# Monash-Connected-Autonomous-Vehicle/unsupervised-pseuso-LiDAR

Measured on AMD Instinct MI355X. Metric: images/sec (fwd+bwd) KITTI 192x640 triplets, full training step, higher is better.
Workload: dtype f32; 1 GPU; BASELINE.json configs[1]: per-GPU batch=12, 192x640 KITTI-shaped triplets, ResNet-18 depth encoder + 6-DoF PoseNet, fp32 (the ResNet trunk's 3x3 stride-1 convolutions and their data gradients: fp32 contractions on split operands -- three bf16 planes per operand, six bf16-MFMA plane products, fp32 accumulation; every other launch: fp32 MFMA), one step = 2x depth fwd + pose fwd + warp/L1/smooth loss; global_batch=12, parallelism=dp1

## Files before the change

### unsupervised-pseuso-lidar_amd/csrc/conv_igemm.hip

```cpp
#include <stdlib.h>
#include <map>
#include <mutex>
#include <type_traits>
#include <utility>

#include "conv_shared.h"
#include "kernel_timer.h"

namespace mcav {

template <class T, int KIND>
__global__ __launch_bounds__(256) void igemm_kernel(IgemmParams p) {
    constexpr int BM = T::BM, BN = T::BN;
    constexpr int CK = T::KD;
    __shared__ __attribute__((aligned(16))) float As[2][BM][T::LD];
    __shared__ __attribute__((aligned(16))) float Bs[2][BN][T::LD];
    __shared__ int s_out[BM];
    __shared__ float s_stat[T::WAVES_M][2][BN];
    constexpr int MAXTAB = 9;
    __shared__ unsigned s_o1[KIND == K_GENERIC ? 1 : MAXTAB][KIND == K_GENERIC ? 1 : BM];
    __shared__ unsigned s_o2[KIND == K_GENERIC ? 1 : MAXTAB][KIND == K_GENERIC ? 1 : BM];
    __shared__ int s_rn[KIND == K_GENERIC ? 1 : BM], s_ry[KIND == K_GENERIC ? 1 : BM], s_rx[KIND == K_GENERIC ? 1 : BM];

    const int tid = threadIdx.x, lane = tid & 63, wave = tid >> 6;
// ... 1251 lines not shown
        maybe_build(t + 1); step(B1{}, B0{}, F1{}, ra0, rb0);
        maybe_build(t + 2); step(B0{}, B1{}, F1{}, ra1, rb1);
        maybe_build(t + 3); step(B1{}, B0{}, F0{}, ra0, rb0);
    } else if (rest == 3) {
        maybe_build(t);     step(B0{}, B1{}, F1{}, ra1, rb1);
        maybe_build(t + 1); step(B1{}, B0{}, F1{}, ra0, rb0);
        maybe_build(t + 2); step(B0{}, B1{}, F0{}, ra1, rb1);
    } else if (rest == 2) {
        maybe_build(t);     step(B0{}, B1{}, F1{}, ra1, rb1);
        maybe_build(t + 1); step(B1{}, B0{}, F0{}, ra0, rb0);
    } else if (rest == 1) {
        maybe_build(t);     step(B0{}, B1{}, F0{}, ra1, rb1);
    }

    constexpr int MF = T::MF;
    const int ccol = lane & (MF - 1);
    float* slab = p.slab + (size_t)split * (p.Ktot + 1) * p.slabN;
    if (do_bias) {
        if (bpix < BPIX) *reinterpret_cast<f32x4*>(&Ys[0][bpix][bcol * 4]) = bsum;
        __syncthreads();
        if (tid < BN) {
            float tsum = 0.f;
            for (int k = 0; k < BPIX; ++k) tsum += Ys[0][k][tid];
            if (n0 + tid < p.slabN) slab[(size_t)p.Ktot * p.slabN + n0 + tid] = tsum;
        }
    }
    const __amdgpu_buffer_rsrc_t rslab = make_rsrc(slab, (unsigned)((size_t)p.Ktot * p.slabN * 4));
    const int rowb = p.slabN * 4;
#pragma unroll
    for (int i = 0; i < T::TM; ++i)
#pragma unroll
        for (int j = 0; j < T::TN; ++j) {
            const int n = n0 + wn0 + j * MF + ccol;
            if (n < p.slabN) {
                const unsigned base = (unsigned)(m0 + wm0 + i * MF + (MF == 32 ? 4 * (lane >> 5) : 4 * (lane >> 4))) * (unsigned)rowb + (unsigned)n * 4u;
#pragma unroll
                for (int r = 0; r < T::ACC; ++r) {
                    const int dr = MF == 32 ? (r & 3) + 8 * (r >> 2) : r;
                    buf_store1(rslab, base + (unsigned)(dr * rowb), acc[i][j][r]);
                }
            }
        }
}

__device__ __forceinline__ void wgrad_presum_body(const float* slab, int splits, size_t elems, int per_group, float* dst, unsigned bx, unsigned by) {
    const size_t e4 = (size_t)bx * 256 + threadIdx.x;
    if (e4 * 4 >= elems) return;
    const int k0 = by * per_group, k1 = min(splits, k0 + per_group);
    const f32x4* src = reinterpret_cast<const f32x4*>(slab) + e4;
    const size_t stride4 = elems / 4;
    f32x4 s0 = {0.f, 0.f, 0.f, 0.f}, s1 = s0, s2 = s0, s3 = s0;
    int k = k0;
    for (; k + 3 < k1; k += 4) {
        s0 += src[(size_t)k * stride4];
        s1 += src[(size_t)(k + 1) * stride4];
        s2 += src[(size_t)(k + 2) * stride4];
        s3 += src[(size_t)(k + 3) * stride4];
    }
    for (; k < k1; ++k) s0 += src[(size_t)k * stride4];
    reinterpret_cast<f32x4*>(dst)[(size_t)by * stride4 + e4] = (s0 + s1) + (s2 + s3);
}

__global__ __launch_bounds__(256) void wgrad_presum_kernel(const float* slab, int splits, size_t elems, int per_group, float* dst) {
    wgrad_presum_body(slab, splits, elems, per_group, dst, blockIdx.x, blockIdx.y);
}

__device__ __forceinline__ void wgrad_reduce_body(float* lds, const float* slab, int splits, int Ktot, int slabN, int Kp, int taps, int Cout, int Cin,
                                                  int CI_T, float* dw, float* dbias, int accumulate, int upm, int Cin_total, int ci_off, int bx, int by) {
    const int co0 = bx * 32, ci0 = by * CI_T;
    const int tx = threadIdx.x & 31, ty = threadIdx.x >> 5;
    const int run = CI_T * taps, stride = run + 1;
    const size_t split_stride = (size_t)(Ktot + 1) * slabN;
    const bool col_ok = co0 + tx < slabN;
    if (upm) {
        for (int idx = ty; idx < run; idx += 8) {
            const int tap = idx / CI_T, r = idx - tap * CI_T, ci = ci0 + r;
            float sum = 0.f;
            if (ci < Cin && col_ok) {
                const int ky = tap / 3, kx = tap - ky * 3;
                for (int cls = 0; cls < 4; ++cls) {
                    const int py = cls >> 1, px = cls & 1;
                    const int ta = py == 0 ? (ky == 0 ? 0 : 1) : (ky == 2 ? 1 : 0), tb = px == 0 ? (kx == 0 ? 0 : 1) : (kx == 2 ? 1 : 0);
                    const float* src = slab + (size_t)((cls * 4 + ta * 2 + tb) * Kp + ci) * slabN + co0 + tx;
                    for (int k = 0; k < splits; ++k) sum += src[(size_t)k * split_stride];
                }
            }
            lds[tx * stride + r * taps + tap] = sum;
        }
    } else {
        for (int idx0 = ty; idx0 < run; idx0 += 32) {
            const float* src[4];
            float sum[4];
            int at[4];
#pragma unroll
            for (int u = 0; u < 4; ++u) {
                const int idx = idx0 + 8 * u, tap = idx / CI_T, r = idx - tap * CI_T;
                const bool ok = idx < run && ci0 + r < Cin && col_ok;
                src[u] = ok ? slab + (size_t)(tap * Kp + ci0 + r) * slabN + co0 + tx : nullptr;
                at[u] = idx < run ? tx * stride + r * taps + tap : -1;
                sum[u] = 0.f;
            }
            int k = 0;
            for (; k + 3 < splits; k += 4) {
                float v[4][4];
#pragma unroll
                for (int u = 0; u < 4; ++u)
#pragma unroll
                    for (int j = 0; j < 4; ++j) v[u][j] = src[u] ? src[u][(size_t)(k + j) * split_stride] : 0.f;
#pragma unroll
                for (int u = 0; u < 4; ++u)
#pragma unroll
                    for (int j = 0; j < 4; ++j) sum[u] += v[u][j];
            }
            for (; k < splits; ++k) {
#pragma unroll
                for (int u = 0; u < 4; ++u) sum[u] += src[u] ? src[u][(size_t)k * split_stride] : 0.f;
            }
#pragma unroll
            for (int u = 0; u < 4; ++u)
                if (at[u] >= 0) lds[at[u]] = sum[u];
        }
    }
    if (dbias && by == 0 && ty == 0 && co0 + tx < Cout) {
        const float* src = slab + (size_t)Ktot * slabN + co0 + tx;
        float sum = 0.f;
        for (int k = 0; k < splits; ++k) sum += src[(size_t)k * split_stride];
        dbias[co0 + tx] = accumulate ? dbias[co0 + tx] + sum : sum;
    }
    __syncthreads();
    const int valid_run = (Cin - ci0 < CI_T ? Cin - ci0 : CI_T) * taps;
    for (int e = threadIdx.x; e < 32 * run; e += 256) {
        const int col = e / run, q = e - col * run;
        if (co0 + col < Cout && q < valid_run) {
            const size_t o = ((size_t)(co0 + col) * Cin_total + ci_off + ci0) * taps + q;
            const float v = lds[col * stride + q];
            dw[o] = accumulate ? dw[o] + v : v;
        }
    }
}

__global__ __launch_bounds__(256) void wgrad_reduce_kernel(const float* slab, int splits, int Ktot, int slabN, int Kp, int taps, int Cout, int Cin,
                                                           int CI_T, float* dw, float* dbias, int accumulate, int upm, int Cin_total, int ci_off) {
    extern __shared__ float lds[];
    wgrad_reduce_body(lds, slab, splits, Ktot, slabN, Kp, taps, Cout, Cin, CI_T, dw, dbias, accumulate, upm, Cin_total, ci_off, blockIdx.x, blockIdx.y);
}

__device__ __forceinline__ int find_item(const mcav_wgrad_reduce_item* items, int n, int blk, bool presum) {
    int lo = 0;
    for (int i = 1; i < n; ++i)
        if ((presum ? items[i].pre_first : items[i].red_first) <= blk) lo = i;
    return lo;
}

__global__ __launch_bounds__(256) void wgrad_presum_multi_kernel(const mcav_wgrad_reduce_item* items, int n) {
    __shared__ int s_i;
    if (threadIdx.x == 0) {
        int best = -1;
        for (int i = 0; i < n; ++i)
            if (items[i].groups > 0 && items[i].pre_first <= (int)blockIdx.x) best = i;
        s_i = best;
    }
    __syncthreads();
    if (s_i < 0) return;
    const mcav_wgrad_reduce_item it = items[s_i];
    const int local = (int)blockIdx.x - it.pre_first;
    if (local >= it.pre_bx * it.groups) return;
    wgrad_presum_body(it.slab, it.splits, (size_t)it.elems, it.per_group, it.pre, (unsigned)(local % it.pre_bx), (unsigned)(local / it.pre_bx));
}

__global__ __launch_bounds__(256) void wgrad_reduce_multi_kernel(const mcav_wgrad_reduce_item* items, int n) {
    extern __shared__ float lds[];
    __shared__ int s_i;
    if (threadIdx.x == 0) s_i = find_item(items, n, (int)blockIdx.x, false);
    __syncthreads();
    const mcav_wgrad_reduce_item it = items[s_i];
    const int local = (int)blockIdx.x - it.red_first;
    if (local >= it.red_gx * it.red_gy) return;
    const float* src = it.groups > 0 ? it.pre : it.slab;
    wgrad_reduce_body(lds, src, it.groups > 0 ? it.groups : it.splits, it.Ktot, it.slabN, it.Kp, it.taps, it.Cout, it.Cin, it.ci_t, it.dw, it.dbias,
                      it.accumulate, it.upm, it.cin_total, it.ci_off, local % it.red_gx, local / it.red_gx);
}

__global__ void pack_weights_kernel(const float* w, int Cout, int Cin, int taps, int transposed, float* packed, int Np, int Kp, int Kstride) {
    const size_t total = (size_t)Np * Kstride;
    for (size_t e = (size_t)blockIdx.x * blockDim.x + threadIdx.x; e < total; e += (size_t)gridDim.x * blockDim.x) {
        const int n = (int)(e / Kstride), kf = (int)(e - (size_t)n * Kstride);
        const int tap = kf / Kp, k = kf - tap * Kp;
        float v = 0.f;
        if (tap < taps) {
            const int co = transposed ? k : n, ci = transposed ? n : k;
            if (co < Cout && ci < Cin) v = w[((size_t)co * Cin + ci) * taps + tap];
        }
        packed[e] = v;
    }
}

struct PackItem {
    const float* src;
    float* dst;
    int Cout, Cin, taps, transposed, Np, Kp, Kstride, first_block;
};

constexpr int PK_LDS = 5120;
constexpr int PK_CO = 64;

__host__ __device__ inline int pack_ci_tile(int taps) { const int t = 79 / taps; return t < 1 ? 1 : (t > 8 ? 8 : t); }

constexpr int PK_MERGE = 2048;

__device__ __forceinline__ float upmerge_elem(const float* w, int Cout, int Cin, int C1, int Np, size_t e) {
    const int c = (int)(e % C1);
    const int mt = (int)((e / C1) % 4), n = (int)((e / ((size_t)C1 * 4)) % Np), cls = (int)(e / ((size_t)C1 * 4 * Np));
    const int py = cls >> 1, px = cls & 1, a = mt >> 1, b = mt & 1;
    float sum = 0.f;
    if (n < Cout) {
        const float* wc = w + ((size_t)n * Cin + c) * 9;
        for (int ky = 0; ky < 3; ++ky)
            for (int kx = 0; kx < 3; ++kx) {
                const bool iny = py == 0 ? (a == 0 ? ky == 0 : ky >= 1) : (a == 0 ? ky <= 1 : ky == 2);
                const bool inx = px == 0 ? (b == 0 ? kx == 0 : kx >= 1) : (b == 0 ? kx <= 1 : kx == 2);
                if (iny && inx) sum += wc[ky * 3 + kx];
            }
    }
    return sum;
}

__device__ __forceinline__ float upmerge_adj_elem(const float* w, int Cout, int Cin, int C1, int Kp, size_t e) {
    const int k = (int)(e % Kp), tap = (int)((e / Kp) % 16), n = (int)(e / ((size_t)Kp * 16));
    const int u = tap >> 2, v = tap & 3;
    float sum = 0.f;
    if (n < C1 && k < Cout) {
        const float* wc = w + ((size_t)k * Cin + n) * 9;
        for (int ky = 0; ky < 3; ++ky)
            for (int kx = 0; kx < 3; ++kx) {
                const bool iny = u == 0 ? ky == 2 : (u == 1 ? ky >= 1 : (u == 2 ? ky <= 1 : ky == 0));
                const bool inx = v == 0 ? kx == 2 : (v == 1 ? kx >= 1 : (v == 2 ? kx <= 1 : kx == 0));
                if (iny && inx) sum += wc[ky * 3 + kx];
            }
    }
    return sum;
}

__host__ __device__ inline size_t pack_merge_total(int transposed, int c1, int Np, int Kp) {
    return (transposed & 16) ? (size_t)Np * 16 * Kp : (size_t)4 * Np * 4 * c1;
}

__host__ __device__ inline int pack_blocks(int transposed, int taps, int Np, int Kp) {
    if (transposed & 24) return (int)((pack_merge_total(transposed, taps, Np, Kp) + PK_MERGE - 1) / PK_MERGE);
    if (!(transposed & 1)) return Np;
    const int ct = pack_ci_tile(taps);
    return ((Np + ct - 1) / ct) * ((Kp + PK_CO - 1) / PK_CO);
}

__global__ __launch_bounds__(256) void pack_weights_multi_kernel(const PackItem* items, int nitems) {
    __shared__ float buf[PK_LDS];
    int lo = 0, hi = nitems - 1;
    while (lo < hi) {
        const int mid = (lo + hi + 1) >> 1;
        if (items[mid].first_block <= (int)blockIdx.x) lo = mid; else hi = mid - 1;
    }
    PackItem it = items[lo];
    if (it.transposed & 24) {
        const size_t total = pack_merge_total(it.transposed, it.taps, it.Np, it.Kp);
        const size_t e0 = (size_t)(blockIdx.x - it.first_block) * PK_MERGE;
        for (int k = 0; k < PK_MERGE / 256; ++k) {
            const size_t e = e0 + (size_t)k * 256 + threadIdx.x;
            if (e < total)
                it.dst[e] = (it.transposed & 16) ? upmerge_adj_elem(it.src, it.Cout, it.Cin, it.taps, it.Kp, e)
                                                 : upmerge_elem(it.src, it.Cout, it.Cin, it.taps, it.Np, e);
        }
        return;
    }
    const bool to_bf16 = (it.transposed & 6) != 0;
    const bool planes = (it.transposed & 4) != 0;
    it.transposed &= 1;
    __bf16* const dst16 = reinterpret_cast<__bf16*>(it.dst);
    const size_t plane = (size_t)it.Np * it.Kstride;
    auto put16 = [&](size_t o, float v) {
        const __bf16 h = (__bf16)v;
        dst16[o] = h;
        if (planes) {
            const float r1 = v - (float)h;
            const __bf16 m = (__bf16)r1;
            dst16[plane + o] = m;
            dst16[2 * plane + o] = (__bf16)(r1 - (float)m);
        }
    };
    const int bl = blockIdx.x - it.first_block, tid = threadIdx.x;
    if (!it.transposed) {
        const int n = bl, run = it.Cin * it.taps;
        float* drow = it.dst + (size_t)n * it.Kstride;
        const bool staged = run <= PK_LDS;
        if (n < it.Cout && staged) {
            const float* srow = it.src + (size_t)n * run;
            for (int q = tid; q < run; q += 256) buf[q] = srow[q];
        }
        __syncthreads();
        for (int kf = tid; kf < it.Kstride; kf += 256) {
            const int tap = kf / it.Kp, k = kf - tap * it.Kp;
            float v = 0.f;
            if (n < it.Cout && tap < it.taps && k < it.Cin) v = staged ? buf[k * it.taps + tap] : it.src[((size_t)n * it.Cin + k) * it.taps + tap];
            if (to_bf16) put16((size_t)n * it.Kstride + kf, v);
            else drow[kf] = v;
        }
        return;
    }
    const int ct = pack_ci_tile(it.taps), run = ct * it.taps, ld = run + 1;
    const int cob = (it.Kp + PK_CO - 1) / PK_CO;
    const int ci0 = (bl / cob) * ct, co0 = (bl % cob) * PK_CO;
    for (int e = tid; e < PK_CO * run; e += 256) {
        const int co = e / run, q = e - co * run;
        float v = 0.f;
        if (co0 + co < it.Cout && ci0 + q / it.taps < it.Cin) v = it.src[((size_t)(co0 + co) * it.Cin + ci0) * it.taps + q];
        buf[co * ld + q] = v;
    }
    __syncthreads();
    for (int e = tid; e < PK_CO * run; e += 256) {
        const int q = e / PK_CO, co = e - q * PK_CO;
        const int r = q / it.taps, tap = q - r * it.taps;
        if (ci0 + r < it.Np && co0 + co < it.Kp) {
            const size_t o = (size_t)(ci0 + r) * it.Kstride + tap * it.Kp + co0 + co;
            if (to_bf16) put16(o, buf[co * ld + q]);
            else it.dst[o] = buf[co * ld + q];
        }
    }
}

__global__ __launch_bounds__(256) void splitk_finish_kernel(const float* __restrict__ slab, int splits, size_t n, int Cd, float* __restrict__ y,
                                                            const float* __restrict__ bias, int n_begin, int act, const float* __restrict__ dact_aux,
                                                            int dact, const float* __restrict__ addend) {
    for (size_t i = (size_t)blockIdx.x * 256 + threadIdx.x; i < n; i += (size_t)gridDim.x * 256) {
        float v = 0.f;
        for (int k = 0; k < splits; ++k) v += slab[(size_t)k * n + i];
        if (bias) v += bias[n_begin + (int)(i % (size_t)Cd)];
        v = act_fwd(v, act);
        if (dact_aux && !(dact & MCAV_DACT_AFTER_ADDEND)) v *= act_bwd(dact_aux[i], dact & 0xff);
        if (addend) v += addend[i];
        if (dact_aux && (dact & MCAV_DACT_AFTER_ADDEND)) v *= act_bwd(dact_aux[i], dact & 0xff);
        y[i] = v;
    }
}

inline float* ksplit_slab(hipStream_t s, size_t bytes) {
    static std::mutex mu;
    static std::map<hipStream_t, std::pair<void*, size_t>> slabs;
    std::lock_guard<std::mutex> lock(mu);
    auto& e = slabs[s];
    if (e.second < bytes) {
        hipStreamCaptureStatus st = hipStreamCaptureStatusNone;
        if (hipStreamIsCapturing(s, &st) != hipSuccess) return nullptr;
        if (st != hipStreamCaptureStatusNone) {
            for (auto& kv : slabs)
                if (kv.second.second >= bytes) return reinterpret_cast<float*>(kv.second.first);
            return nullptr;
        }
        void* ptr = nullptr;
        if (hipMalloc(&ptr, bytes) != hipSuccess) return nullptr;
        e = {ptr, bytes};
    }
    return reinterpret_cast<float*>(e.first);
}

template <class T, int ID>
inline void launch_igemm(const IgemmRoute& r, hipStream_t s) {
    static_assert(T::BM == tile_bm(ID) && T::BN == tile_bn(ID) && T::KD == tile_kd(ID) && T::AROWS == tile_arows(ID), "conv_plan.h's tile table");
    IgemmParams p = r.p;
    if (r.ksplit > 1) {
        float* slab = ksplit_slab(s, (size_t)p.g.B * p.Hd * p.Wd * p.Cd * 4 * r.ksplit);
        if (slab) { p.ksplit = r.ksplit; p.kslab = slab; }
    }
    const int grid = p.mtiles * p.ntiles * p.ksplit;
    const size_t tab_bytes = sizeof(unsigned) * (size_t)p.taps * T::BM * (p.g.C2 > 0 ? 2 : 1);
    const size_t refl_bytes = sizeof(unsigned) * (size_t)p.taps * T::BM * 4;
    switch (r.variant) {
        case MCAV_RV_TABLE | MCAV_RV_UPM: timed_launch(igemm_tab_kernel<T, 2>, grid, dim3(256), sizeof(unsigned) * 13 * T::BM, s, p); break;
        case MCAV_RV_TABLE: timed_launch(igemm_tab_kernel<T, 0>, grid, dim3(256), tab_bytes, s, p); break;
        case MCAV_RV_TABLE | MCAV_RV_REFLECT | MCAV_RV_ADJ: timed_launch(igemm_tab_kernel<T, 1>, grid, dim3(256), refl_bytes, s, p); break;
        case MCAV_RV_FAST: timed_launch(igemm_kernel<T, K_FAST>, grid, dim3(256), 0, s, p); break;
// ... 65 lines not shown
MCAV_EXPORT int mcav_igemm(const mcav_igemm_desc* d, void* stream) {
    IgemmRoute r;
    const int rc = plan_igemm(d, plan_env(), r);
    if (rc != MCAV_OK) return rc;
    hipStream_t s = as_stream(stream);
    switch (r.family) {
        case MCAV_IGEMM_HALO: mcav_halo_launch(r, s); break;
        case MCAV_IGEMM_STEM: mcav_stem_launch(r, s); break;
        case MCAV_IGEMM_FP32:
            switch (r.tile) {
                case 1: launch_igemm<Tile128x64, 1>(r, s); break;
                case 2: launch_igemm<Tile64x64, 2>(r, s); break;
                case 3: launch_igemm<Tile256x32, 3>(r, s); break;
                case 4: launch_igemm<Tile256x16, 4>(r, s); break;
                case 5: launch_igemm<Tile128x128, 5>(r, s); break;
                case 6: launch_igemm<Tile64x16, 6>(r, s); break;
                case 7: launch_igemm<Tile128x32, 7>(r, s); break;
                case 8: launch_igemm<Tile128x64k32, 8>(r, s); break;
                case 9: launch_igemm<Tile128x128k32, 9>(r, s); break;
                case 10: launch_igemm<Tile64x64k32, 10>(r, s); break;
                case 11: launch_igemm<Tile64x64k64, 11>(r, s); break;
                case 12: launch_igemm<Tile32x64k32, 12>(r, s); break;
                default: return MCAV_E_INVALID;
            }
            break;
        default: return mcav_patch_bf16_launch(r, s);
    }
    return launch_status();
}

MCAV_EXPORT int mcav_wgrad_route(const mcav_wgrad_desc* d, mcav_conv_route* out) {
    if (!out) return MCAV_E_INVALID;
    *out = mcav_conv_route{};
    WgradRoute r;
    const int rc = plan_wgrad_route(d, plan_env(), r);
    const WgradParams& p = r.pl.p;
    if (rc == MCAV_OK)
        *out = mcav_conv_route{r.family, r.variant, r.pl.tile, p.mtiles, p.ntiles, r.workgroups, p.splits, r.workspace_bytes()};
    return rc;
}

MCAV_EXPORT size_t mcav_wgrad_workspace_bytes(const mcav_wgrad_desc* d) {
    WgradRoute r;
    return plan_wgrad_route(d, plan_env(), r) == MCAV_OK ? r.workspace_bytes() : 0;
}

MCAV_EXPORT int mcav_wgrad_uses_bf16(const mcav_wgrad_desc* d) {
    WgradRoute r;
    return plan_wgrad_route(d, plan_env(), r) == MCAV_OK && (r.family == MCAV_WGRAD_BF16_PATCH || r.family == MCAV_WGRAD_BF16_TILE);
}

static int wgrad_gemm(const mcav_wgrad_desc* d, void* workspace, size_t workspace_bytes, hipStream_t s, WgradRoute& r) {
    if (plan_wgrad_route(d, plan_env(), r) != MCAV_OK || !workspace) return MCAV_E_INVALID;
    if (workspace_bytes < r.workspace_bytes()) return MCAV_E_WORKSPACE;
    r.pl.p.slab = reinterpret_cast<float*>(workspace);
    switch (r.family) {
        case MCAV_WGRAD_BF16_PATCH:
        case MCAV_WGRAD_BF16_TILE: mcav_bf16_wgrad_launch(r.pl.p, s); break;
        case MCAV_WGRAD_STEM: mcav_stem_wgrad_launch(r, s); break;
        case MCAV_WGRAD_HALO: mcav_halo_wgrad_launch(r, s); break;
        default:
            switch (r.pl.tile) {
                case 1: launch_wgrad<Tile128x64, 1>(r, s); break;
                case 2: launch_wgrad<Tile64x64, 2>(r, s); break;
                case 3: launch_wgrad<Tile256x32, 3>(r, s); break;
                case 4: launch_wgrad<Tile256x16, 4>(r, s); break;
                case 6: launch_wgrad<Tile64x16, 6>(r, s); break;
                case 7: launch_wgrad<Tile128x32, 7>(r, s); break;
                default: return MCAV_E_INVALID;
            }
    }
    return MCAV_OK;
}

static void fill_reduce_item(const mcav_wgrad_desc* d, const WgradPlan& pl, void* workspace, mcav_wgrad_reduce_item& it) {
    it.slab = pl.p.slab;
    it.pre = pl.groups ? reinterpret_cast<float*>(reinterpret_cast<char*>(workspace) + pl.slab_bytes) : nullptr;
    it.dw = d->dw_oihw;
    it.dbias = d->dbias;
    it.elems = (unsigned long long)(pl.p.Ktot + 1) * pl.p.slabN;
    it.splits = pl.p.splits; it.groups = pl.groups; it.per_group = pl.per_group;
    it.Ktot = pl.p.Ktot; it.slabN = pl.p.slabN; it.Kp = pl.p.Kp;
    it.taps = pl.p.upm ? 9 : pl.p.taps;
    it.Cout = d->Cout; it.Cin = d->Cin; it.ci_t = pl.ci_t;
    it.accumulate = d->accumulate; it.upm = pl.p.upm;
    it.cin_total = d->Cin_total > 0 ? d->Cin_total : d->Cin;
    it.ci_off = d->ci_offset;
    it.pre_bx = pl.groups ? (int)((it.elems / 4 + 255) / 256) : 0;
    it.red_gx = (d->Cout + 31) / 32;
    it.red_gy = (d->Cin + pl.ci_t - 1) / pl.ci_t;
    it.pre_first = 0; it.red_first = 0;
}

MCAV_EXPORT int mcav_wgrad(const mcav_wgrad_desc* d, void* workspace, size_t workspace_bytes, void* stream) {
    WgradRoute r;
    hipStream_t s = as_stream(stream);
    const int rc = wgrad_gemm(d, workspace, workspace_bytes, s, r);
    if (rc != MCAV_OK) return rc;
    mcav_wgrad_reduce_item it;
    fill_reduce_item(d, r.pl, workspace, it);
    const size_t lds_bytes = sizeof(float) * 32 * (size_t)(it.ci_t * it.taps + 1);
    const float* rsrc = it.slab;
    int rsplits = it.splits;
    if (it.groups) {
        timed_launch(wgrad_presum_kernel, dim3((unsigned)it.pre_bx, it.groups), dim3(256), 0, s, (const float*)it.slab, it.splits, (size_t)it.elems,
                     it.per_group, it.pre);
// ... 102 lines not shown
```

### unsupervised-pseuso-lidar_amd/mcav/nn.py

```python
import ctypes
import os
import os as _os

import torch

from . import lib as L

c_p, c_i, c_f, c_sz, c_d = L.c_p, L.c_i, L.c_f, L.c_sz, ctypes.c_double

G_DIRECT, G_SMALLC, G_ADJ_REFLECT, G_ADJ_STRIDE2 = 0, 1, 2, 3
PAD_ZERO, PAD_REFLECT = 0, 1
ACT_NONE, ACT_RELU, ACT_ELU, ACT_SIGMOID = 0, 1, 2, 3
DACT_AFTER_ADDEND = 0x100
TILE_ID_MASK = 0xff
TILE_GENERAL = 1 << 9
TILE_HALO_9TAP = 1 << 10
TILE_NO_UPMERGE = 1 << 11
TILE_ALT_UPMERGE = 1 << 12


class IgemmDesc(ctypes.Structure):
    _fields_ = [("x1", c_p), ("x2", c_p), ("B", c_i), ("Hs", c_i), ("Ws", c_i), ("C1", c_i), ("C2", c_i), ("up1", c_i),
                ("w", c_p), ("kh", c_i), ("kw", c_i), ("Np", c_i), ("Kp", c_i),
                ("mode", c_i), ("stride", c_i), ("sign", c_i), ("offset", c_i), ("pad_mode", c_i),
# ... 143 lines not shown
        return False


def _planned(d):
    r = ConvRoute()
    (L.lib().mcav_igemm_route if isinstance(d, IgemmDesc) else L.lib().mcav_wgrad_route)(ctypes.byref(d), ctypes.byref(r))
    return r


def _stem_executed(flops, cout):
    return flops * (8.0 / 7.0) * (1.0 if cout >= 32 else 2.0)


def up16(v):
    return (v + 15) // 16 * 16


def empty(shape, like):
    return torch.empty(shape, dtype=torch.float32, device=like.device)


def P(t):
    return t.data_ptr() if t is not None else None


class _PackItem(ctypes.Structure):
    _fields_ = [("src", c_p), ("dst", c_p), ("Cout", c_i), ("Cin", c_i), ("taps", c_i), ("transposed", c_i), ("Np", c_i), ("Kp", c_i),
                ("Kstride", c_i), ("first_block", c_i)]


MMA_FP32, MMA_BF16, MMA_SPLIT, MMA_SPLIT_ALL = 0, 1, 2, 3
DEFAULT_MMA = MMA_SPLIT
_KINDS = {"f": (False, 0), "b": (True, 0), "f16": (False, 1), "b16": (True, 1), "f16s": (False, 3), "b16s": (True, 3)}


class PackRegistry:

    def __init__(self):
        self.entries = []
        self.table = None
        self.retired = []
        self.nblocks = 0
        self.signature = None

    def add(self, spec, kind):
        import weakref
        self.entries.append((weakref.ref(spec), kind))
        self.signature = None

    def _build(self, device, live):
        items = (_PackItem * len(live))()
        blk = 0
        for it, (spec, kind) in zip(items, live):
            if kind in ("um", "ua"):
                buf = spec._packs[kind]
                it.src, it.dst = spec.weight.data_ptr(), buf.data_ptr()
                it.Cout, it.Cin, it.taps = spec.cout, spec.cin, spec._merge_c1
                if kind == "um":
                    it.transposed, it.Np, it.Kp = 8, spec.np, 0
                else:
                    it.transposed, it.Np, it.Kp = 16, buf.shape[0], buf.shape[1] // 16
                it.Kstride, it.first_block = 0, blk
                blk += L.lib().mcav_pack_weights_blocks(it.taps, it.transposed, it.Np, max(it.Kp, 1))
                continue
            tr, h = _KINDS[kind]
            buf = spec._packs[kind]
            np_, kp_ = (up16(spec.cin), up16(spec.cout)) if tr else (spec.np, spec.kp)
            it.src, it.dst = spec.weight.data_ptr(), buf.data_ptr()
            it.Cout, it.Cin, it.taps, it.transposed = spec.cout, spec.cin, spec.kh * spec.kw, int(tr) | (4 if h == 3 else 2 if h else 0)
            it.Np, it.Kp, it.Kstride, it.first_block = np_, kp_, buf.shape[1], blk
            blk += L.lib().mcav_pack_weights_blocks(it.taps, int(tr), np_, kp_)
        raw = torch.frombuffer(bytearray(bytes(items)), dtype=torch.uint8)
        if self.table is not None:
            self.retired.append(self.table)
        self.table = raw.to(device)
        self.nblocks = blk

    def repack_all(self, device):
        self.entries = [(r, k) for r, k in self.entries if r() is not None]
        live = [(r(), k) for r, k in self.entries]
        live = [(s, k) for s, k in live if s is not None and s.weight.device == device and s._packs.get(k) is not None]
        if not live:
            return
        sig = tuple((s.weight.data_ptr(), s._packs[k].data_ptr()) for s, k in live)
        if self.table is None or sig != self.signature or self.table.device != device:
            self._build(device, live)
            self.signature = sig
        L.check(L.lib().mcav_pack_weights_multi(P(self.table), len(live), self.nblocks, L.stream()), "mcav_pack_weights_multi")
        for s, k in live:
            s._keys[k] = s._key()


PACKS = PackRegistry()


def refresh_packed_weights(device):
    for ref, k in PACKS.entries:
        s = ref()
        if s is None or s.weight.device != device:
            continue
        if s._keys.get(k) != s._key():
            PACKS.repack_all(device)
            return


class ConvSpec:

    def __init__(self, weight, bias, stride, pad, pad_mode, smallc=False):
        self.weight, self.bias = weight, bias
        self.cout, self.cin, self.kh, self.kw = weight.shape
        self.stride, self.pad, self.pad_mode = stride, pad, pad_mode
        self.smallc = smallc
        self.kp = 4 if smallc else up16(self.cin)
        self.np = up16(self.cout)
# ... 8 lines not shown
        tr, h = _KINDS[kind]
        key = self._key()
        buf = self._packs.get(kind)
        if buf is None or self._keys.get(kind) != key or buf.device != self.weight.device:
            taps = self.kh * self.kw
            if buf is None or buf.device != self.weight.device:
                shape = (up16(self.cin), taps * up16(self.cout)) if tr else (self.np, up16(taps * self.kp))
                buf = torch.empty((shape[0] * max(h, 1), shape[1]), dtype=torch.bfloat16 if h else torch.float32, device=self.weight.device)
                f32 = torch.empty(shape, dtype=torch.float32, device=self.weight.device) if h else buf
                np_, kp_ = (up16(self.cin), up16(self.cout)) if tr else (self.np, self.kp)
                L.check(L.lib().mcav_pack_weights(P(self.weight), self.cout, self.cin, self.kh, self.kw, int(tr), P(f32), np_, kp_, L.stream()),
                        "mcav_pack_weights")
                if h == 3:
                    L.check(L.lib().mcav_f32_to_bf16_planes(P(f32), P(buf), f32.numel(), L.stream()), "mcav_f32_to_bf16_planes")
                elif h:
                    L.check(L.lib().mcav_f32_to_bf16(P(f32), P(buf), f32.numel(), L.stream()), "mcav_f32_to_bf16")
                self._packs[kind] = buf
                self._keys[kind] = key
                PACKS.add(self, kind)
            else:
                PACKS.repack_all(self.weight.device)
        return self._packs[kind]

    def packed_fwd(self):
        return self._packed("f")

    def packed_bwd(self):
        return self._packed("b")

    def packed_fwd16(self):
        return self._packed("f16")

    def packed_bwd16(self):
        return self._packed("b16")

    def packed_fwd16s(self):
        return self._packed("f16s")

    def packed_bwd16s(self):
        return self._packed("b16s")

    def is_stem(self):
        return ((self.kh, self.kw, self.stride, self.pad, self.pad_mode) == (7, 7, 2, 3, PAD_ZERO)
                and ((self.smallc and (self.cout, self.cin) == (64, 3)) or (not self.smallc and (self.cout, self.cin) == (16, 9))))

    def takes_stem(self, x2, up1, tile):
        return self.is_stem() and x2 is None and not up1 and not tile & TILE_GENERAL

    def fwd_gather(self):
        return (G_SMALLC if self.smallc else G_DIRECT, self.stride, 1, -self.pad, self.pad_mode)

    def packed_stem(self):
        key = self._key()
        if getattr(self, "_stem", None) is None or self._key_s != key or self._stem.device != self.weight.device:
            if getattr(self, "_stem", None) is None or self._stem.device != self.weight.device:
                self._stem = empty((self.cin * 56, self.cout), self.weight)
            L.check(L.lib().mcav_pack_stem_weights(P(self.weight), self.cout, self.cin, P(self._stem), L.stream()), "mcav_pack_stem_weights")
            self._key_s = key
        return self._stem

    def packed_upmerge(self, c1):
        return self._merged("um", c1, lambda: empty((4, self.np, 4, c1), self.weight),
                            lambda buf: L.lib().mcav_pack_weights_upmerge(P(self.weight), self.cout, self.cin, c1, P(buf), self.np, L.stream()))

    def _merged(self, kind, c1, make, pack):
        key = self._key()
        buf = self._packs.get(kind)
        if buf is None or buf.device != self.weight.device or getattr(self, "_merge_c1", c1) != c1:
            if buf is not None and getattr(self, "_merge_c1", c1) != c1:
                raise L.MCAVError("a convolution's merged-tap copies are built for ONE split of its input channels (got %d after %d)" % (c1, self._merge_c1))
            self._merge_c1 = c1
            first = buf is None
            buf = self._packs[kind] = make()
            L.check(pack(buf), "mcav_pack_weights_upmerge(%s)" % kind)
            self._keys[kind] = key
            if first:
                PACKS.add(self, kind)
        elif self._keys.get(kind) != key:
            PACKS.repack_all(self.weight.device)
        return self._packs[kind]

    def packed_upmerge_adj(self, c1, bf16=False):
        npd, kpd = up16(c1), up16(self.cout)
        upa = self._merged("ua", c1, lambda: empty((npd, 16 * kpd), self.weight),
                           lambda buf: L.lib().mcav_pack_weights_upmerge_adj(P(self.weight), self.cout, self.cin, c1, P(buf), npd, kpd, L.stream()))
        self._upa = upa
        key = self._key() + (c1,)
        if not bf16:
            return self._upa
        planes = 3 if bf16 == 3 else 1
        if getattr(self, "_upa16", None) is None or self._key_ua16 != key or self._upa16.shape[0] != planes * self._upa.shape[0]:
            if getattr(self, "_upa16", None) is None or self._upa16.shape[0] != planes * self._upa.shape[0]:
                self._upa16 = torch.empty((planes * self._upa.shape[0], self._upa.shape[1]), dtype=torch.bfloat16, device=self._upa.device)
            if planes == 3:
                L.check(L.lib().mcav_f32_to_bf16_planes(P(self._upa), P(self._upa16), self._upa.numel(), L.stream()), "mcav_f32_to_bf16_planes")
            else:
                L.check(L.lib().mcav_f32_to_bf16(P(self._upa), P(self._upa16), self._upa.numel(), L.stream()), "mcav_f32_to_bf16")
            self._key_ua16 = key
        return self._upa16


SPLIT_WGRAD = _os.environ.get("MCAV_SPLIT_WGRAD", "0") != "0"
SPLIT_NAMES = ("fp32-split", "fp32_split", "f32s", "fp32s")
MFMA32_NAMES = ("fp32-mfma", "fp32_mfma", "f32-mfma")


def set_compute_dtype(module, dtype):
    bf16 = dtype in (torch.bfloat16, "bf16", "bfloat16")
    split = dtype in SPLIT_NAMES
    pinned = dtype in MFMA32_NAMES
    if not bf16 and not split and not pinned and dtype not in (torch.float32, "fp32", "f32", "float32", None):
        raise L.MCAVError("compute dtype must be fp32, fp32-mfma, fp32-split or bf16, got %r" % (dtype,))
    mma = MMA_BF16 if bf16 else MMA_SPLIT if split else MMA_FP32 if pinned else DEFAULT_MMA
    for m in module.modules():
        if hasattr(m, "weight") and getattr(m, "weight") is not None and m.weight.dim() == 4:
            m._mcav_mma = mma
            spec = getattr(m, "_mcav_spec", None)
            if spec is not None:
                spec.mma = m._mcav_mma
    return module


STEM_PLANAR = _os.environ.get("MCAV_STEM_PLANAR", "1") != "0"
PLANAR_BATCH, PLANAR_CHANNELS = 1, 2


class PlanarImages:

    def __init__(self, images, stack, cp):
        images = [L.dev(t.contiguous(), "image") for t in images]
        if not 1 <= len(images) <= 3 or any(t.shape != images[0].shape or t.dtype != torch.float32 for t in images) or images[0].shape[1] != 3:
            raise L.MCAVError("PlanarImages: one to three float32 [B,3,H,W] image batches of one shape")
        if stack == PLANAR_CHANNELS and len(images) != 3:
            raise L.MCAVError("PlanarImages: the channel-stacked form takes three images")
        self.images, self.stack, self.cp = images, stack, cp
        Bp, _, H, W = images[0].shape
        self.shape = (Bp * (len(images) if stack == PLANAR_BATCH else 1), H, W, cp)
        self.device, self.is_cuda = images[0].device, images[0].is_cuda

    def numel(self):
        return sum(t.numel() for t in self.images)

    def fill(self, d):
        d.x1 = None
        for i, t in enumerate(self.images):
            d.x_planar[i] = P(t)
        d.planar_B, d.planar_stack = self.images[0].shape[0], self.stack

    def packed(self):
        if self.stack == PLANAR_CHANNELS:
            return nchw3_to_nhwc(self.images[0], self.images[1], self.images[2], self.cp)
# ... 687 lines not shown
```

Measured before the change: 1134 images/s.

## Vectorize wgrad reductions and weight packing; batch stem and bf16 upmerge packs

The weight-gradient presum and reduce kernels now use nontemporal vector loads, with each thread summing four output columns as f32x4 instead of scalars. The upmerge and non-upmerge paths share one loop, and dw is written back with 16-byte stores when alignment allows. Item lookup in the multi-kernels becomes a per-thread binary search with no shared-memory sync. Weight packing uses vectorized 4-wide and 8-wide bf16 stores, and the stem and bf16 upmerge packs move into the batched multi-pack launch so they no longer need separate launches. This is meant to cut memory-bound reduction and packing time and launch count, at the cost of new alignment requirements and more complex indexing.

Result: no change. 1139 images/s (median of 5 runs) (+0.5%).

```diff
diff --git a/unsupervised-pseuso-lidar_amd/csrc/conv_igemm.hip b/unsupervised-pseuso-lidar_amd/csrc/conv_igemm.hip
--- a/unsupervised-pseuso-lidar_amd/csrc/conv_igemm.hip
+++ b/unsupervised-pseuso-lidar_amd/csrc/conv_igemm.hip
@@ -1327,12 +1327,12 @@
     f32x4 s0 = {0.f, 0.f, 0.f, 0.f}, s1 = s0, s2 = s0, s3 = s0;
     int k = k0;
     for (; k + 3 < k1; k += 4) {
-        s0 += src[(size_t)k * stride4];
-        s1 += src[(size_t)(k + 1) * stride4];
-        s2 += src[(size_t)(k + 2) * stride4];
-        s3 += src[(size_t)(k + 3) * stride4];
-    }
-    for (; k < k1; ++k) s0 += src[(size_t)k * stride4];
+        s0 += __builtin_nontemporal_load(src + (size_t)k * stride4);
+        s1 += __builtin_nontemporal_load(src + (size_t)(k + 1) * stride4);
+        s2 += __builtin_nontemporal_load(src + (size_t)(k + 2) * stride4);
+        s3 += __builtin_nontemporal_load(src + (size_t)(k + 3) * stride4);
+    }
+    for (; k < k1; ++k) s0 += __builtin_nontemporal_load(src + (size_t)k * stride4);
     reinterpret_cast<f32x4*>(dst)[(size_t)by * stride4 + e4] = (s0 + s1) + (s2 + s3);
 }
 
@@ -1346,64 +1346,102 @@
     const int tx = threadIdx.x & 31, ty = threadIdx.x >> 5;
     const int run = CI_T * taps, stride = run + 1;
     const size_t split_stride = (size_t)(Ktot + 1) * slabN;
-    const bool col_ok = co0 + tx < slabN;
-    if (upm) {
-        for (int idx = ty; idx < run; idx += 8) {
-            const int tap = idx / CI_T, r = idx - tap * CI_T, ci = ci0 + r;
-            float sum = 0.f;
-            if (ci < Cin && col_ok) {
-                const int ky = tap / 3, kx = tap - ky * 3;
-                for (int cls = 0; cls < 4; ++cls) {
-                    const int py = cls >> 1, px = cls & 1;
+    const int c4 = threadIdx.x & 7, rw = threadIdx.x >> 3;
+    const bool col_ok = co0 + 4 * c4 < slabN;
+    const int ncls = upm ? 4 : 1;
+    for (int idx0 = rw; idx0 < run; idx0 += 128) {
+        f32x4 sum[4];
+        int at[4], tap[4], ci[4];
+        bool ok[4];
+#pragma unroll
+        for (int u = 0; u < 4; ++u) {
+            const int idx = idx0 + 32 * u, r = idx - (idx / CI_T) * CI_T;
+            tap[u] = idx / CI_T;
+            ci[u] = ci0 + r;
+            ok[u] = idx < run && ci[u] < Cin && col_ok;
+            at[u] = idx < run ? r * taps + tap[u] : -1;
+            sum[u] = f32x4{0.f, 0.f, 0.f, 0.f};
+        }
+        for (int cls = 0; cls < ncls; ++cls) {
+            const f32x4* src[4];
+#pragma unroll
+            for (int u = 0; u < 4; ++u) {
+                int row = tap[u] * Kp + ci[u];
+                if (upm) {
+                    const int ky = tap[u] / 3, kx = tap[u] - ky * 3, py = cls >> 1, px = cls & 1;
                     const int ta = py == 0 ? (ky == 0 ? 0 : 1) : (ky == 2 ? 1 : 0), tb = px == 0 ? (kx == 0 ? 0 : 1) : (kx == 2 ? 1 : 0);
-                    const float* src = slab + (size_t)((cls * 4 + ta * 2 + tb) * Kp + ci) * slabN + co0 + tx;
-                    for (int k = 0; k < splits; ++k) sum += src[(size_t)k * split_stride];
+                    row = (cls * 4 + ta * 2 + tb) * Kp + ci[u];
                 }
-            }
-            lds[tx * stride + r * taps + tap] = sum;
-        }
-    } else {
-        for (int idx0 = ty; idx0 < run; idx0 += 32) {
-            const float* src[4];
-            float sum[4];
-            int at[4];
-#pragma unroll
-            for (int u = 0; u < 4; ++u) {
-                const int idx = idx0 + 8 * u, tap = idx / CI_T, r = idx - tap * CI_T;
-                const bool ok = idx < run && ci0 + r < Cin && col_ok;
-                src[u] = ok ? slab + (size_t)(tap * Kp + ci0 + r) * slabN + co0 + tx : nullptr;
-                at[u] = idx < run ? tx * stride + r * taps + tap : -1;
-                sum[u] = 0.f;
-            }
+                src[u] = reinterpret_cast<const f32x4*>(ok[u] ? slab + (size_t)row * slabN + co0 + 4 * c4 : slab);
+            }
+            const size_t ss4 = split_stride / 4;
             int k = 0;
             for (; k + 3 < splits; k += 4) {
-                float v[4][4];
+                f32x4 v[4][4];
 #pragma unroll
                 for (int u = 0; u < 4; ++u)
 #pragma unroll
-                    for (int j = 0; j < 4; ++j) v[u][j] = src[u] ? src[u][(size_t)(k + j) * split_stride] : 0.f;
+                    for (int j = 0; j < 4; ++j) v[u][j] = __builtin_nontemporal_load(src[u] + (size_t)(k + j) * ss4);
 #pragma unroll
                 for (int u = 0; u < 4; ++u)
 #pragma unroll
                     for (int j = 0; j < 4; ++j) sum[u] += v[u][j];
             }
             for (; k < splits; ++k) {
-#pragma unroll
-                for (int u = 0; u < 4; ++u) sum[u] += src[u] ? src[u][(size_t)k * split_stride] : 0.f;
-            }
-#pragma unroll
-            for (int u = 0; u < 4; ++u)
-                if (at[u] >= 0) lds[at[u]] = sum[u];
-        }
+                f32x4 v[4];
+#pragma unroll
+                for (int u = 0; u < 4; ++u) v[u] = __builtin_nontemporal_load(src[u] + (size_t)k * ss4);
+#pragma unroll
+                for (int u = 0; u < 4; ++u) sum[u] += v[u];
+            }
+        }
+#pragma unroll
+        for (int u = 0; u < 4; ++u)
+            if (at[u] >= 0) {
+#pragma unroll
+                for (int j = 0; j < 4; ++j) lds[(4 * c4 + j) * stride + at[u]] = ok[u] ? sum[u][j] : 0.f;
+            }
     }
     if (dbias && by == 0 && ty == 0 && co0 + tx < Cout) {
         const float* src = slab + (size_t)Ktot * slabN + co0 + tx;
         float sum = 0.f;
-        for (int k = 0; k < splits; ++k) sum += src[(size_t)k * split_stride];
+        for (int k = 0; k < splits; k += 8) {
+            float v[8];
+#pragma unroll
+            for (int j = 0; j < 8; ++j) v[j] = src[(size_t)min(k + j, splits - 1) * split_stride];
+#pragma unroll
+            for (int j = 0; j < 8; ++j)
+                if (k + j < splits) sum += v[j];
+        }
         dbias[co0 + tx] = accumulate ? dbias[co0 + tx] + sum : sum;
     }
     __syncthreads();
     const int valid_run = (Cin - ci0 < CI_T ? Cin - ci0 : CI_T) * taps;
+    const size_t row_stride = (size_t)Cin_total * taps, base = ((size_t)co0 * Cin_total + ci_off + ci0) * taps;
+    if (!(valid_run & 3) && !(row_stride & 3) && !(base & 3) && !(reinterpret_cast<size_t>(dw) & 15)) {
+        const int rq = valid_run >> 2, total = (Cout - co0 < 32 ? Cout - co0 : 32) * rq;
+        for (int e0 = threadIdx.x; e0 < total; e0 += 1024) {
+            f32x4 v[4], old[4];
+            f32x4* at[4];
+#pragma unroll
+            for (int u = 0; u < 4; ++u) {
+                const int e = e0 + 256 * u < total ? e0 + 256 * u : e0, col = e / rq, q = (e - col * rq) * 4;
+                const float* l = lds + col * stride + q;
+                v[u] = f32x4{l[0], l[1], l[2], l[3]};
+                at[u] = reinterpret_cast<f32x4*>(dw + base + (size_t)col * row_stride + q);
+            }
+            if (accumulate) {
+#pragma unroll
+                for (int u = 0; u < 4; ++u) old[u] = *at[u];
+#pragma unroll
+                for (int u = 0; u < 4; ++u) v[u] = old[u] + v[u];
+            }
+#pragma unroll
+            for (int u = 0; u < 4; ++u)
+                if (e0 + 256 * u < total) *at[u] = v[u];
+        }
+        return;
+    }
     for (int e = threadIdx.x; e < 32 * run; e += 256) {
         const int col = e / run, q = e - col * run;
         if (co0 + col < Cout && q < valid_run) {
@@ -1421,36 +1459,27 @@
 }
 
 __device__ __forceinline__ int find_item(const mcav_wgrad_reduce_item* items, int n, int blk, bool presum) {
-    int lo = 0;
-    for (int i = 1; i < n; ++i)
-        if ((presum ? items[i].pre_first : items[i].red_first) <= blk) lo = i;
+    int lo = 0, hi = n - 1;
+    while (lo < hi) {
+        const int mid = (lo + hi + 1) >> 1;
+        if ((presum ? items[mid].pre_first : items[mid].red_first) <= blk) lo = mid; else hi = mid - 1;
+    }
     return lo;
 }
 
 __global__ __launch_bounds__(256) void wgrad_presum_multi_kernel(const mcav_wgrad_reduce_item* items, int n) {
-    __shared__ int s_i;
-    if (threadIdx.x == 0) {
-        int best = -1;
-        for (int i = 0; i < n; ++i)
-            if (items[i].groups > 0 && items[i].pre_first <= (int)blockIdx.x) best = i;
-        s_i = best;
-    }
-    __syncthreads();
-    if (s_i < 0) return;
-    const mcav_wgrad_reduce_item it = items[s_i];
+    const mcav_wgrad_reduce_item it = items[find_item(items, n, (int)blockIdx.x, true)];
+    if (it.groups <= 0) return;
     const int local = (int)blockIdx.x - it.pre_first;
-    if (local >= it.pre_bx * it.groups) return;
+    if (local < 0 || local >= it.pre_bx * it.groups) return;
     wgrad_presum_body(it.slab, it.splits, (size_t)it.elems, it.per_group, it.pre, (unsigned)(local % it.pre_bx), (unsigned)(local / it.pre_bx));
 }
 
 __global__ __launch_bounds__(256) void wgrad_reduce_multi_kernel(const mcav_wgrad_reduce_item* items, int n) {
     extern __shared__ float lds[];
-    __shared__ int s_i;
-    if (threadIdx.x == 0) s_i = find_item(items, n, (int)blockIdx.x, false);
-    __syncthreads();
-    const mcav_wgrad_reduce_item it = items[s_i];
+    const mcav_wgrad_reduce_item it = items[find_item(items, n, (int)blockIdx.x, false)];
     const int local = (int)blockIdx.x - it.red_first;
-    if (local >= it.red_gx * it.red_gy) return;
+    if (local < 0 || local >= it.red_gx * it.red_gy) return;
     const float* src = it.groups > 0 ? it.pre : it.slab;
     wgrad_reduce_body(lds, src, it.groups > 0 ? it.groups : it.splits, it.Ktot, it.slabN, it.Kp, it.taps, it.Cout, it.Cin, it.ci_t, it.dw, it.dbias,
                       it.accumulate, it.upm, it.cin_total, it.ci_off, local % it.red_gx, local / it.red_gx);
@@ -1516,15 +1545,146 @@
     return sum;
 }
 
+__device__ __forceinline__ float stem_elem(const float* w, int Cout, int Cin, size_t e) {
+    const int n = (int)(e % Cout), k = (int)(e / Cout);
+    const int hh = k & 1, j = (k >> 1) & 3, cky = k >> 3, ky = cky % 7, c = cky / 7;
+    const int kx = 2 * j + hh;
+    return kx < 7 ? w[(((size_t)n * Cin + c) * 7 + ky) * 7 + kx] : 0.f;
+}
+
 __host__ __device__ inline size_t pack_merge_total(int transposed, int c1, int Np, int Kp) {
+    if (transposed & 32) return (size_t)Np * Kp;
     return (transposed & 16) ? (size_t)Np * 16 * Kp : (size_t)4 * Np * 4 * c1;
 }
 
 __host__ __device__ inline int pack_blocks(int transposed, int taps, int Np, int Kp) {
-    if (transposed & 24) return (int)((pack_merge_total(transposed, taps, Np, Kp) + PK_MERGE - 1) / PK_MERGE);
+    if (transposed & 56) return (int)((pack_merge_total(transposed, taps, Np, Kp) + PK_MERGE - 1) / PK_MERGE);
     if (!(transposed & 1)) return Np;
     const int ct = pack_ci_tile(taps);
     return ((Np + ct - 1) / ct) * ((Kp + PK_CO - 1) / PK_CO);
+}
+
+typedef __bf16 pk_bf16x8 __attribute__((ext_vector_type(8)));
+
+struct PackOut {
+    float* f32;
+    __bf16* b16;
+    size_t plane;
+    bool planes;
+    bool wide;
+};
+
+template <int W>
+__device__ __forceinline__ void pack_store(const PackOut& d, size_t o, const float (&v)[W], int nv) {
+    if constexpr (W == 4) {
+        if (d.wide && nv == W) *reinterpret_cast<f32x4*>(d.f32 + o) = f32x4{v[0], v[1], v[2], v[3]};
+        else
+            for (int j = 0; j < nv; ++j) d.f32[o + j] = v[j];
+    } else {
+        pk_bf16x8 h, m, l;
+#pragma unroll
+        for (int j = 0; j < W; ++j) {
+            const __bf16 hj = (__bf16)v[j];
+            const float r1 = v[j] - (float)hj;
+            const __bf16 mj = (__bf16)r1;
+            h[j] = hj;
+            m[j] = mj;
+            l[j] = (__bf16)(r1 - (float)mj);
+        }
+        if (d.wide && nv == W) {
+            *reinterpret_cast<pk_bf16x8*>(d.b16 + o) = h;
+            if (d.planes) {
+                *reinterpret_cast<pk_bf16x8*>(d.b16 + d.plane + o) = m;
+                *reinterpret_cast<pk_bf16x8*>(d.b16 + 2 * d.plane + o) = l;
+            }
+        } else {
+            for (int j = 0; j < nv; ++j) {
+                d.b16[o + j] = h[j];
+                if (d.planes) {
+                    d.b16[d.plane + o + j] = m[j];
+                    d.b16[2 * d.plane + o + j] = l[j];
+                }
+            }
+        }
+    }
+}
+
+template <int W>
+__device__ __forceinline__ void pack_forward_row(const PackItem& it, const PackOut& out, float* buf, int n, int tid) {
+    const int run = it.Cin * it.taps, ldc = it.Cin | 1;
+    const bool live = n < it.Cout, staged = (long)it.taps * ldc <= PK_LDS;
+    if (live && staged) {
+        const float* srow = it.src + (size_t)n * run;
+        const int dk = 256 / it.taps, dt = 256 - dk * it.taps;
+        int k = tid / it.taps, tap = tid - k * it.taps;
+        for (int q0 = tid; q0 < run; q0 += 8 * 256) {
+            float v[8];
+#pragma unroll
+            for (int j = 0; j < 8; ++j) v[j] = srow[q0 + 256 * j < run ? q0 + 256 * j : q0];
+#pragma unroll
+            for (int j = 0; j < 8; ++j) {
+                if (q0 + 256 * j < run) buf[tap * ldc + k] = v[j];
+                k += dk;
+                tap += dt;
+                if (tap >= it.taps) { tap -= it.taps; ++k; }
+            }
+        }
+    }
+    __syncthreads();
+    for (int kf = tid * W; kf < it.Kstride; kf += 256 * W) {
+        int tap = kf / it.Kp, k = kf - tap * it.Kp;
+        float v[W];
+#pragma unroll
+        for (int j = 0; j < W; ++j) {
+            float x = 0.f;
+            if (live && tap < it.taps && k < it.Cin) x = staged ? buf[tap * ldc + k] : it.src[((size_t)n * it.Cin + k) * it.taps + tap];
+            v[j] = x;
+            if (++k == it.Kp) { k = 0; ++tap; }
+        }
+        pack_store<W>(out, (size_t)n * it.Kstride + kf, v, it.Kstride - kf < W ? it.Kstride - kf : W);
+    }
+}
+
+template <int W>
+__device__ __forceinline__ void pack_transposed_tile(const PackItem& it, const PackOut& out, float* buf, int bl, int tid) {
+    const int ct = pack_ci_tile(it.taps), run = ct * it.taps, ld = run + 1;
+    const int cob = (it.Kp + PK_CO - 1) / PK_CO;
+    const int ci0 = (bl / cob) * ct, co0 = (bl % cob) * PK_CO;
+    const int qlim = it.Cin > ci0 ? (it.Cin - ci0 < ct ? (it.Cin - ci0) * it.taps : run) : 0;
+    {
+        const int dco = 256 / run, dq = 256 - dco * run;
+        int co = tid / run, q = tid - co * run;
+        for (int e0 = tid; e0 < PK_CO * run; e0 += 8 * 256) {
+            float v[8];
+            int at[8];
+#pragma unroll
+            for (int j = 0; j < 8; ++j) {
+                const bool ok = e0 + 256 * j < PK_CO * run && co0 + co < it.Cout && q < qlim;
+                v[j] = it.src[ok ? ((size_t)(co0 + co) * it.Cin + ci0) * it.taps + q : 0];
+                if (!ok) v[j] = 0.f;
+                at[j] = e0 + 256 * j < PK_CO * run ? co * ld + q : -1;
+                co += dco;
+                q += dq;
+                if (q >= run) { q -= run; ++co; }
+            }
+#pragma unroll
+            for (int j = 0; j < 8; ++j)
+                if (at[j] >= 0) buf[at[j]] = v[j];
+        }
+    }
+    __syncthreads();
+    constexpr int CPR = PK_CO / W;
+    for (int e = tid; e < run * CPR; e += 256) {
+        const int q = e / CPR, c = (e - q * CPR) * W;
+        const int r = q / it.taps, tap = q - r * it.taps;
+        const int nv = it.Kp - co0 - c < W ? it.Kp - co0 - c : W;
+        if (ci0 + r < it.Np && nv > 0) {
+            float v[W];
+#pragma unroll
+            for (int j = 0; j < W; ++j) v[j] = buf[(c + j) * ld + q];
+            pack_store<W>(out, (size_t)(ci0 + r) * it.Kstride + tap * it.Kp + co0 + c, v, nv);
+        }
+    }
 }
 
 __global__ __launch_bounds__(256) void pack_weights_multi_kernel(const PackItem* items, int nitems) {
@@ -1535,70 +1695,47 @@
         if (items[mid].first_block <= (int)blockIdx.x) lo = mid; else hi = mid - 1;
     }
     PackItem it = items[lo];
-    if (it.transposed & 24) {
+    if (it.transposed & 56) {
         const size_t total = pack_merge_total(it.transposed, it.taps, it.Np, it.Kp);
         const size_t e0 = (size_t)(blockIdx.x - it.first_block) * PK_MERGE;
+        __bf16* const dst16 = reinterpret_cast<__bf16*>(it.dst);
         for (int k = 0; k < PK_MERGE / 256; ++k) {
             const size_t e = e0 + (size_t)k * 256 + threadIdx.x;
-            if (e < total)
-                it.dst[e] = (it.transposed & 16) ? upmerge_adj_elem(it.src, it.Cout, it.Cin, it.taps, it.Kp, e)
+            if (e >= total) continue;
+            const float v = (it.transposed & 32) ? stem_elem(it.src, it.Cout, it.Cin, e)
+                          : (it.transposed & 16) ? upmerge_adj_elem(it.src, it.Cout, it.Cin, it.taps, it.Kp, e)
                                                  : upmerge_elem(it.src, it.Cout, it.Cin, it.taps, it.Np, e);
+            if (it.transposed & 6) {
+                const __bf16 h = (__bf16)v;
+                dst16[e] = h;
+                if (it.transposed & 4) {
+                    const float r1 = v - (float)h;
+                    const __bf16 m = (__bf16)r1;
+                    dst16[total + e] = m;
+                    dst16[2 * total + e] = (__bf16)(r1 - (float)m);
+                }
+            } else {
+                it.dst[e] = v;
+            }
         }
         return;
     }
     const bool to_bf16 = (it.transposed & 6) != 0;
-    const bool planes = (it.transposed & 4) != 0;
-    it.transposed &= 1;
-    __bf16* const dst16 = reinterpret_cast<__bf16*>(it.dst);
-    const size_t plane = (size_t)it.Np * it.Kstride;
-    auto put16 = [&](size_t o, float v) {
-        const __bf16 h = (__bf16)v;
-        dst16[o] = h;
-        if (planes) {
-            const float r1 = v - (float)h;
-            const __bf16 m = (__bf16)r1;
-            dst16[plane + o] = m;
-            dst16[2 * plane + o] = (__bf16)(r1 - (float)m);
-        }
-    };
+    PackOut out;
+    out.f32 = it.dst;
+    out.b16 = reinterpret_cast<__bf16*>(it.dst);
+    out.plane = (size_t)it.Np * it.Kstride;
+    out.planes = (it.transposed & 4) != 0;
     const int bl = blockIdx.x - it.first_block, tid = threadIdx.x;
-    if (!it.transposed) {
-        const int n = bl, run = it.Cin * it.taps;
-        float* drow = it.dst + (size_t)n * it.Kstride;
-        const bool staged = run <= PK_LDS;
-        if (n < it.Cout && staged) {
-            const float* srow = it.src + (size_t)n * run;
-            for (int q = tid; q < run; q += 256) buf[q] = srow[q];
-        }
-        __syncthreads();
-        for (int kf = tid; kf < it.Kstride; kf += 256) {
-            const int tap = kf / it.Kp, k = kf - tap * it.Kp;
-            float v = 0.f;
-            if (n < it.Cout && tap < it.taps && k < it.Cin) v = staged ? buf[k * it.taps + tap] : it.src[((size_t)n * it.Cin + k) * it.taps + tap];
-            if (to_bf16) put16((size_t)n * it.Kstride + kf, v);
-            else drow[kf] = v;
-        }
+    if (!(it.transposed & 1)) {
+        out.wide = (reinterpret_cast<size_t>(it.dst) & 15) == 0 && it.Kstride % 16 == 0;
+        if (to_bf16) pack_forward_row<8>(it, out, buf, bl, tid);
+        else pack_forward_row<4>(it, out, buf, bl, tid);
         return;
     }
-    const int ct = pack_ci_tile(it.taps), run = ct * it.taps, ld = run + 1;
-    const int cob = (it.Kp + PK_CO - 1) / PK_CO;
-    const int ci0 = (bl / cob) * ct, co0 = (bl % cob) * PK_CO;
-    for (int e = tid; e < PK_CO * run; e += 256) {
-        const int co = e / run, q = e - co * run;
-        float v = 0.f;
-        if (co0 + co < it.Cout && ci0 + q / it.taps < it.Cin) v = it.src[((size_t)(co0 + co) * it.Cin + ci0) * it.taps + q];
-        buf[co * ld + q] = v;
-    }
-    __syncthreads();
-    for (int e = tid; e < PK_CO * run; e += 256) {
-        const int q = e / PK_CO, co = e - q * PK_CO;
-        const int r = q / it.taps, tap = q - r * it.taps;
-        if (ci0 + r < it.Np && co0 + co < it.Kp) {
-            const size_t o = (size_t)(ci0 + r) * it.Kstride + tap * it.Kp + co0 + co;
-            if (to_bf16) put16(o, buf[co * ld + q]);
-            else it.dst[o] = buf[co * ld + q];
-        }
-    }
+    out.wide = (reinterpret_cast<size_t>(it.dst) & 15) == 0 && it.Kstride % 16 == 0 && it.Kp % 8 == 0;
+    if (to_bf16) pack_transposed_tile<8>(it, out, buf, bl, tid);
+    else pack_transposed_tile<4>(it, out, buf, bl, tid);
 }
 
 __global__ __launch_bounds__(256) void splitk_finish_kernel(const float* __restrict__ slab, int splits, size_t n, int Cd, float* __restrict__ y,
@@ -1770,6 +1907,7 @@
 
 static int wgrad_gemm(const mcav_wgrad_desc* d, void* workspace, size_t workspace_bytes, hipStream_t s, WgradRoute& r) {
     if (plan_wgrad_route(d, plan_env(), r) != MCAV_OK || !workspace) return MCAV_E_INVALID;
+    if (reinterpret_cast<size_t>(workspace) & 15) return MCAV_E_INVALID;
     if (workspace_bytes < r.workspace_bytes()) return MCAV_E_WORKSPACE;
     r.pl.p.slab = reinterpret_cast<float*>(workspace);
     switch (r.family) {
diff --git a/unsupervised-pseuso-lidar_amd/mcav/nn.py b/unsupervised-pseuso-lidar_amd/mcav/nn.py
--- a/unsupervised-pseuso-lidar_amd/mcav/nn.py
+++ b/unsupervised-pseuso-lidar_amd/mcav/nn.py
@@ -219,14 +219,21 @@
         items = (_PackItem * len(live))()
         blk = 0
         for it, (spec, kind) in zip(items, live):
-            if kind in ("um", "ua"):
+            if kind in ("um", "ua", "ua16", "st"):
                 buf = spec._packs[kind]
                 it.src, it.dst = spec.weight.data_ptr(), buf.data_ptr()
-                it.Cout, it.Cin, it.taps = spec.cout, spec.cin, spec._merge_c1
-                if kind == "um":
-                    it.transposed, it.Np, it.Kp = 8, spec.np, 0
+                it.Cout, it.Cin = spec.cout, spec.cin
+                if kind == "st":
+                    it.taps, it.transposed, it.Np, it.Kp = spec.kh * spec.kw, 32, spec.cin * 56, spec.cout
                 else:
-                    it.transposed, it.Np, it.Kp = 16, buf.shape[0], buf.shape[1] // 16
+                    it.taps = spec._merge_c1
+                    if kind == "um":
+                        it.transposed, it.Np, it.Kp = 8, spec.np, 0
+                    elif kind == "ua":
+                        it.transposed, it.Np, it.Kp = 16, buf.shape[0], buf.shape[1] // 16
+                    else:
+                        rows = up16(spec._merge_c1)
+                        it.transposed, it.Np, it.Kp = 16 | (4 if buf.shape[0] == 3 * rows else 2), rows, buf.shape[1] // 16
                 it.Kstride, it.first_block = 0, blk
                 blk += L.lib().mcav_pack_weights_blocks(it.taps, it.transposed, it.Np, max(it.Kp, 1))
                 continue
@@ -341,11 +348,17 @@
 
     def packed_stem(self):
         key = self._key()
-        if getattr(self, "_stem", None) is None or self._key_s != key or self._stem.device != self.weight.device:
-            if getattr(self, "_stem", None) is None or self._stem.device != self.weight.device:
-                self._stem = empty((self.cin * 56, self.cout), self.weight)
-            L.check(L.lib().mcav_pack_stem_weights(P(self.weight), self.cout, self.cin, P(self._stem), L.stream()), "mcav_pack_stem_weights")
-            self._key_s = key
+        buf = self._packs.get("st")
+        if buf is None or buf.device != self.weight.device:
+            first = buf is None
+            buf = self._packs["st"] = empty((self.cin * 56, self.cout), self.weight)
+            L.check(L.lib().mcav_pack_stem_weights(P(self.weight), self.cout, self.cin, P(buf), L.stream()), "mcav_pack_stem_weights")
+            self._keys["st"] = key
+            if first:
+                PACKS.add(self, "st")
+        elif self._keys.get("st") != key:
+            PACKS.repack_all(self.weight.device)
+        self._stem = self._packs["st"]
         return self._stem
 
     def packed_upmerge(self, c1):
@@ -374,18 +387,25 @@
         upa = self._merged("ua", c1, lambda: empty((npd, 16 * kpd), self.weight),
                            lambda buf: L.lib().mcav_pack_weights_upmerge_adj(P(self.weight), self.cout, self.cin, c1, P(buf), npd, kpd, L.stream()))
         self._upa = upa
-        key = self._key() + (c1,)
         if not bf16:
             return self._upa
         planes = 3 if bf16 == 3 else 1
-        if getattr(self, "_upa16", None) is None or self._key_ua16 != key or self._upa16.shape[0] != planes * self._upa.shape[0]:
-            if getattr(self, "_upa16", None) is None or self._upa16.shape[0] != planes * self._upa.shape[0]:
-                self._upa16 = torch.empty((planes * self._upa.shape[0], self._upa.shape[1]), dtype=torch.bfloat16, device=self._upa.device)
+        buf = self._packs.get("ua16")
+        if buf is None or buf.device != upa.device or buf.shape[0] != planes * upa.shape[0]:
+            first = buf is None
+            buf = self._packs["ua16"] = torch.empty((planes * upa.shape[0], upa.shape[1]), dtype=torch.bfloat16, device=upa.device)
             if planes == 3:
-                L.check(L.lib().mcav_f32_to_bf16_planes(P(self._upa), P(self._upa16), self._upa.numel(), L.stream()), "mcav_f32_to_bf16_planes")
+                L.check(L.lib().mcav_f32_to_bf16_planes(P(upa), P(buf), upa.numel(), L.stream()), "mcav_f32_to_bf16_planes")
             else:
-                L.check(L.lib().mcav_f32_to_bf16(P(self._upa), P(self._upa16), self._upa.numel(), L.stream()), "mcav_f32_to_bf16")
-            self._key_ua16 = key
+                L.check(L.lib().mcav_f32_to_bf16(P(upa), P(buf), upa.numel(), L.stream()), "mcav_f32_to_bf16")
+            self._keys["ua16"] = self._key()
+            if first:
+                PACKS.add(self, "ua16")
+            else:
+                PACKS.signature = None
+        elif self._keys.get("ua16") != self._key():
+            PACKS.repack_all(self.weight.device)
+        self._upa16 = self._packs["ua16"]
         return self._upa16
 
 
```
